# YoungSeng/DiffuseStyleGesture

Hardware: AMD Instinct MI355X
Metric: gesture frames/sec, 1000-step DDPM, 320-frame ZEGGS clip, 1/2/4/8 MI355X (higher is better)
Workload: dtype bf16

## Files before the change

diffusestylegesture_amd/csrc/dsg_fused.h:

```cpp
#pragma once
#include "dsg_kernels.h"

namespace dsg {

struct InLocArgs {
    const void* xs;
    int Jp;
    const void* Wp;
    int KBtot;
    LocArgs loc;
    StepCtl* ctl_upd;
    StepTables st; int n_tab;
};

template <class P, int HD, int W>
__device__ __forceinline__ void inloc_body(const InLocArgs& g) {
    typedef typename P::elem elem;
    constexpr int ES = (int)sizeof(elem);
    preload_kernargs(g);
    const LocArgs& a = g.loc;
    if (blockIdx.z == gridDim.z - 1) {
        if (g.ctl_upd && blockIdx.x == 0 && blockIdx.y == 0 && threadIdx.x == 0) step_advance_B<P>(g.ctl_upd, g.st, g.n_tab);
        return;
    }
// ... 994 lines not shown
#pragma unroll
            for (int e = 0; e < 4; ++e) { pp[e] = f2bf(s[2 * kb][e]); pp[4 + e] = f2bf(s[2 * kb + 1][e]); }
            pfr[kb] = __builtin_bit_cast(f32x4, pp);
        }
    }
    const int q = qt * 16 + lr;
#pragma unroll
    for (int dt = 0; dt < ND; ++dt) {
        f32x4 o = (f32x4){0.f, 0.f, 0.f, 0.f};
#pragma unroll
        for (int kb = 0; kb < NVF; ++kb) o = P::mma(vs[dt * NVF + kb][lane], pfr[kb], o);
        if (q < g.ntok) {
            f32x4 y;
#pragma unroll
            for (int e = 0; e < 4; ++e) y[e] = o[e] * inv;
            P::store4_afrag((elem*)g.out, (size_t)qk_off<P>(b * g.ntok + q, h * HD + dt * 16 + 4 * lg, KD), y);
        }
    }
    DSG_TL_MARK(7);
}

struct FfnArgs {
    const void* A;
    const float* R;
    const void* W1; const float* b1;
    const void* W2; const float* b2;
    const float* ln_g; const float* ln_b;
    float* Xn;
    void* Xa;
    int M, MT;
    const void* Wo; const float* bo;
    const float* ln1_g; const float* ln1_b;
    float* X1;
};

template <class P, int DT, int FT, int RT, int NW, int LA = 2, bool LATE_R = false, bool OP = false, int RING = 0, bool WO_RING = false>
__global__ __launch_bounds__(64 * NW) void k_ffn(const FfnArgs g) {
    DSG_TL_SCOPE();
    typedef typename P::elem elem;
    constexpr int ES = (int)sizeof(elem);
    constexpr int D = 64 * DT, FF = 64 * FT, KD = D / P::KB, KF = FF / P::KB;
    constexpr int FW = FF / 16 / NW, DW = D / 16 / NW;
    constexpr int HP = FF * ES + 16;
    constexpr int KC0 = (DW >= 4 ? 2 : 4) * LA, KC = KC0 < KF ? KC0 : KF, NC = KF / KC;
    constexpr int NT = 64 * NW;
    static_assert(FW >= LA && FW % LA == 0 && DW >= 1 && KF % KC == 0 && (FF / 16) % NW == 0 && (D / 16) % NW == 0, "shape");
    static_assert(!P::W2 || (OP && RING > 0 && RT < 4), "bf16w2: the ring forms with the prologue");
    constexpr int HID_LO = RT * 16 * HP;
    __shared__ __attribute__((aligned(16))) char hid[P::AF * RT * 16 * HP];
    __shared__ float red[RT][2][NW][16];
    __shared__ __attribute__((aligned(16))) float vecs[3][D];
    constexpr int XP = D * ES + 16;
    constexpr bool BIG = OP && RT >= 4;
    constexpr bool X1MEM = BIG || (OP && RT == 2 && D >= 512);
    static_assert(!BIG || RT * 16 * XP <= RT * 16 * HP, "alias");
    constexpr int XA_LO = RT * 16 * XP;
    __shared__ __attribute__((aligned(16))) char xa_own[(OP && !BIG) ? P::AF * RT * 16 * XP : 16];
    char* const xa = BIG ? hid : xa_own;
    __shared__ __attribute__((aligned(16))) float vecs1[OP ? 3 : 1][OP ? D : 4];
    constexpr int X1P = D + 4;
    __shared__ __attribute__((aligned(16))) float x1f[(OP && !X1MEM) ? RT * 16 * X1P : 4];
    preload_kernargs(g);
    const int mb = blockIdx.x;
    const int tid = threadIdx.x, lane = tid & 63, wave = wave_id(), lr = lane & 15, lg = lane >> 4;
    const int m0 = mb * 16 * RT, mt_last = g.MT - 1;
    constexpr int RH = (OP && RT >= 4) ? 2 : RT;
    typename P::afrag af[RT][KD];
    constexpr int NFH = RH * KD, NFW = (NFH + NW - 1) / NW;
    f32x4* const stg = (f32x4*)(hid + P::AF * (RT * 16 * HP - NFH * 1024));
    static_assert(!OP || NFH * 1024 + (RT >= 4 ? RT * 16 * (D * ES + 16) : 0) <= RT * 16 * HP, "the staged fragments sit behind the (aliased) LayerNorm1 rows");
    typename P::afrag afw[OP ? NFW : 1];
    auto load_a = [&](int rt0) {
        if constexpr (OP) {
#pragma unroll
            for (int i = 0; i < NFW; ++i) {
                const int f = min(wave * NFW + i, NFH - 1), rt = rt0 + f / KD, kb = f % KD;
                const int mt = min(mb * RT + rt, mt_last);
                afw[i] = P::aload_frag(g.A, (size_t)(mt * KD + kb), lane);
            }
        } else {
#pragma unroll
            for (int rt = rt0; rt < rt0 + RH; ++rt) {
                const int mt = min(mb * RT + rt, mt_last);
#pragma unroll
                for (int kb = 0; kb < KD; ++kb) af[rt][kb] = P::aload_frag(g.A, (size_t)(mt * KD + kb), lane);
            }
        }
    };
    auto share_a = [&](int rt0) {
#pragma unroll
        for (int i = 0; i < NFW; ++i) if (wave * NFW + i < NFH) {
            if constexpr (P::W2) { stg[((wave * NFW + i) * 2) * 64 + lane] = afw[i].h; stg[((wave * NFW + i) * 2 + 1) * 64 + lane] = afw[i].l; }
            else stg[(wave * NFW + i) * 64 + lane] = afw[i];
        }
        DSG_LDS_BARRIER();
#pragma unroll
        for (int rt = rt0; rt < rt0 + RH; ++rt)
#pragma unroll
            for (int kb = 0; kb < KD; ++kb) af[rt][kb] = P::aload((const char*)&stg[((rt - rt0) * KD + kb) * P::AF * 64 + lane], 1024);
    };
    load_a(0);
    const f32x4* w1 = (const f32x4*)g.W1 + lane;
    const f32x4* w2 = (const f32x4*)g.W2 + lane;
    f32x4 wb1[2][LA][KD], pb1[2][LA];
    auto load1 = [&](int buf, int tp) {
#pragma unroll
        for (int j = 0; j < LA; ++j) {
            const int nt = wave * FW + LA * tp + j;
#pragma unroll
            for (int kb = 0; kb < KD; ++kb) wb1[buf][j][kb] = w1[((size_t)nt * KD + kb) * 64];
            pb1[buf][j] = *(const f32x4*)(g.b1 + nt * 16 + 4 * lg);
        }
    };
    constexpr int N0 = WO_RING ? DW * KD : 0;
    constexpr int N1 = FW * KD, N2 = KF * DW, NRING = RING > 0 ? RING : 1;
    static_assert(RING == 0 || (OP && RING <= N1), "ring");
    static_assert(!WO_RING || (RING > 0 && RING <= N0 && RT <= 2), "W_o in the ring: the 16- and 32-row forms");
    typename P::wfrag ring[NRING];
    const f32x4* wo_ring = (const f32x4*)g.Wo + lane;
    auto ring_load = [&](int ig) -> typename P::wfrag {
        if (ig < N0) return P::wload(wo_ring, (size_t)(wave * DW + ig % DW) * KD + ig / DW);
        const int i = ig - N0;
        if (i < N1) return P::wload(w1, (size_t)(wave * FW + i / KD) * KD + i % KD);
        const int k = (i - N1) / DW, t = (i - N1) % DW;
        return P::wload(w2, (size_t)(wave * DW + t) * KF + k);
    };
    if constexpr (!OP) load1(0, 0);
    f32x4 pr[RT][DW];
    auto rowok_of = [&](int rt) { return m0 + rt * 16 + lr < g.M; };
    auto mrow_of = [&](int rt) { return (unsigned)min(m0 + rt * 16 + lr, g.M - 1); };
#pragma unroll
    for (int rt = 0; rt < RT; ++rt) {
        if ((!LATE_R || OP) && rt < RH) {
#pragma unroll
            for (int t = 0; t < DW; ++t) pr[rt][t] = lda16<P>(g.R, (size_t)((mrow_of(rt) * D + (wave * DW + t) * 16 + 4 * lg) * 4u));
        }
    }
    constexpr int NV = (3 * D / 4 + NT - 1) / NT;
    f32x4 vload[NV], vload1[OP ? NV : 1];
#pragma unroll
    for (int i = 0; i < NV; ++i) {
        const int e = min(tid + NT * i, 3 * D / 4 - 1), vsel = e / (D / 4), vidx = e % (D / 4);
        vload[i] = ((const f32x4*)(vsel == 0 ? g.b2 : (vsel == 1 ? g.ln_g : g.ln_b)))[vidx];
        if constexpr (OP) vload1[i] = ((const f32x4*)(vsel == 0 ? g.bo : (vsel == 1 ? g.ln1_g : g.ln1_b)))[vidx];
    }
    if constexpr (OP) {
        const f32x4* wo = (const f32x4*)g.Wo + lane;
        typename P::wfrag wof[WO_RING ? 1 : DW][WO_RING ? 1 : KD];
        if constexpr (WO_RING) {
#pragma unroll
            for (int i = 0; i < RING; ++i) ring[i] = ring_load(i);
        } else {
#pragma unroll
            for (int t = 0; t < DW; ++t)
#pragma unroll
                for (int kb = 0; kb < KD; ++kb) wof[t][kb] = P::wload(wo, (size_t)(wave * DW + t) * KD + kb);
        }
        DSG_LOADS_ISSUED();
// ... 81 lines not shown
                const int n = (wave * DW + t) * 16 + 4 * lg;
                const f32x4 pg = *(const f32x4*)(&vecs1[1][n]), pbt = *(const f32x4*)(&vecs1[2][n]);
                f32x4 y;
#pragma unroll
                for (int e = 0; e < 4; ++e) y[e] = __builtin_fmaf((acc1[rt][t][e] - mean1[rt]) * rstd, pg[e], pbt[e]);
                P::store4_a((elem*)(xa + (rt * 16 + lr) * XP) + n, XA_LO, y);
                if constexpr (X1MEM) *(f32x4*)((char*)g.X1 + (size_t)(((unsigned)(m0 + rt * 16 + lr) * D + n) * 4u)) = y;
                else *(f32x4*)(x1f + (rt * 16 + lr) * X1P + n) = y;
            }
        }
        if constexpr (RING > 0 && !WO_RING) {
#pragma unroll
            for (int i = 3 * (RING / 4); i < RING; ++i) ring[i] = ring_load(i);
            DSG_LOADS_ISSUED();
        }
        DSG_LDS_BARRIER();
#pragma unroll
        for (int rt = 0; rt < RT; ++rt)
#pragma unroll
            for (int kb = 0; kb < KD; ++kb) af[rt][kb] = P::aload(xa + (rt * 16 + lr) * XP + (kb * P::KB + P::E * lg) * ES, XA_LO);
        if constexpr (BIG) DSG_LDS_BARRIER();
        DSG_TL_MARK(2);
    } else {
        DSG_LOADS_ISSUED();
    }
    f32x4 acc[RT][DW];
#pragma unroll
    for (int rt = 0; rt < RT; ++rt)
#pragma unroll
        for (int t = 0; t < DW; ++t) acc[rt][t] = (f32x4){0.f, 0.f, 0.f, 0.f};
    if constexpr (RING > 0) {
        static_assert(OP, "ring: the forms with the prologue");
        f32x4 pbr[2];
        pbr[0] = *(const f32x4*)(g.b1 + (wave * FW) * 16 + 4 * lg);
#pragma unroll
        for (int j = 0; j < FW; ++j) {
            const int nt = wave * FW + j;
            if (j + 1 < FW) pbr[(j + 1) & 1] = *(const f32x4*)(g.b1 + (nt + 1) * 16 + 4 * lg);
            f32x4 c[RT];
#pragma unroll
            for (int rt = 0; rt < RT; ++rt) c[rt] = (f32x4){0.f, 0.f, 0.f, 0.f};
#pragma unroll
            for (int kb = 0; kb < KD; ++kb) {
                const int i = N0 + j * KD + kb;
#pragma unroll
                for (int rt = 0; rt < RT; ++rt) c[rt] = P::mma_w(ring[i % NRING], af[rt][kb], c[rt]);
                if (i + RING < N0 + N1 + N2) ring[i % NRING] = ring_load(i + RING);
                DSG_LOADS_ISSUED();
            }
#pragma unroll
            for (int rt = 0; rt < RT; ++rt) {
                f32x4 y;
#pragma unroll
                for (int e = 0; e < 4; ++e) y[e] = gelu_erf<P>(c[rt][e] + pbr[j & 1][e]);
                P::store4_a((elem*)(hid + (rt * 16 + lr) * HP) + nt * 16 + 4 * lg, HID_LO, y);
            }
        }
        if constexpr (X1MEM) {
            int lr_late = lr;
#ifndef DSG_EMU
            asm volatile("" : "+v"(lr_late));
#endif
#pragma unroll
            for (int rt = 0; rt < RT; ++rt)
#pragma unroll
                for (int t = 0; t < DW; ++t) pr[rt][t] = lda16<P>((const float*)g.X1, (size_t)(((unsigned)(m0 + rt * 16 + lr_late) * D + (wave * DW + t) * 16 + 4 * lg) * 4u));
        }
        DSG_TL_MARK(3);
        DSG_LDS_BARRIER();
        DSG_TL_MARK(4);
        constexpr int AB = RT <= 2 ? 2 : 1;
        typename P::afrag a[AB][RT];
        if constexpr (AB == 2) {
#pragma unroll
            for (int rt = 0; rt < RT; ++rt) a[0][rt] = P::aload(hid + (rt * 16 + lr) * HP + (P::E * lg) * ES, HID_LO);
        }
#pragma unroll
        for (int k = 0; k < KF; ++k) {
            if (AB == 1 || k + 1 < KF) {
                const int kn = AB == 2 ? k + 1 : k;
#pragma unroll
                for (int rt = 0; rt < RT; ++rt) a[kn % AB][rt] = P::aload(hid + (rt * 16 + lr) * HP + (kn * P::KB + P::E * lg) * ES, HID_LO);
            }
#pragma unroll
            for (int t = 0; t < DW; ++t) {
                const int i = N0 + N1 + k * DW + t;
#pragma unroll
                for (int rt = 0; rt < RT; ++rt) acc[rt][t] = P::mma_w(ring[i % NRING], a[k % AB][rt], acc[rt][t]);
                if (i + RING < N0 + N1 + N2) ring[i % NRING] = ring_load(i + RING);
            }
            DSG_LOADS_ISSUED();
        }
    } else {
    #pragma unroll
        for (int tp = 0; tp < FW / LA; ++tp) {
            if (tp + 1 < FW / LA) { load1((tp + 1) & 1, tp + 1); DSG_LOADS_ISSUED(); }
    #pragma unroll
            for (int j = 0; j < LA; ++j) {
                const int nt = wave * FW + LA * tp + j;
    #pragma unroll
                for (int rt = 0; rt < RT; ++rt) {
                    f32x4 c = (f32x4){0.f, 0.f, 0.f, 0.f};
    #pragma unroll
                    for (int kb = 0; kb < KD; ++kb) c = P::mma(wb1[tp & 1][j][kb], af[rt][kb], c);
                    f32x4 y;
    #pragma unroll
                    for (int e = 0; e < 4; ++e) y[e] = gelu_erf<P>(c[e] + pb1[tp & 1][j][e]);
                    P::store4((elem*)(hid + (rt * 16 + lr) * HP) + nt * 16 + 4 * lg, y);
                }
            }
        }
// ... 13 lines not shown
    #endif
            }
    #pragma unroll
            for (int rt = 0; rt < RT; ++rt) {
                const unsigned mr = X1MEM ? (unsigned)(m0 + rt * 16 + lr_late) : (unsigned)min(m0 + rt * 16 + lr_late, g.M - 1);
    #pragma unroll
                for (int t = 0; t < DW; ++t) pr[rt][t] = lda16<P>(X1MEM ? (const float*)g.X1 : g.R, (size_t)((mr * D + (wave * DW + t) * 16 + 4 * lg) * 4u));
            }
        }
        DSG_LOADS_ISSUED();
        if constexpr (!OP) {
    #pragma unroll
            for (int i = 0; i < NV; ++i) {
                const int e = tid + NT * i;
                if (e < 3 * D / 4) *(f32x4*)(&vecs[0][0] + e * 4) = vload[i];
            }
        }
        DSG_LDS_BARRIER();
    #pragma unroll
        for (int c = 0; c < NC; ++c) {
            if (c + 1 < NC) { load2((c + 1) & 1, c + 1); DSG_LOADS_ISSUED(); }
    #pragma unroll
            for (int k = 0; k < KC; ++k) {
    #pragma unroll
                for (int rt = 0; rt < RT; ++rt) {
                    const f32x4 a = *(const f32x4*)(hid + (rt * 16 + lr) * HP + ((c * KC + k) * P::KB + P::E * lg) * ES);
    #pragma unroll
                    for (int t = 0; t < DW; ++t) acc[rt][t] = P::mma(wb2[c & 1][k][t], a, acc[rt][t]);
                }
            }
        }
    }
    DSG_TL_MARK(5);
#pragma unroll
    for (int rt = 0; rt < RT; ++rt) {
        float sm = 0.f;
#pragma unroll
        for (int t = 0; t < DW; ++t) {
            const f32x4 pb = *(const f32x4*)(&vecs[0][(wave * DW + t) * 16 + 4 * lg]);
            if constexpr (OP && !X1MEM) pr[rt][t] = *(const f32x4*)(x1f + (rt * 16 + lr) * X1P + (wave * DW + t) * 16 + 4 * lg);
            acc[rt][t] = acc[rt][t] + pb + pr[rt][t];
            sm += (acc[rt][t][0] + acc[rt][t][1]) + (acc[rt][t][2] + acc[rt][t][3]);
        }
        ln_wave_moments<DW>(acc[rt], sm, red[rt][0][wave], red[rt][1][wave], lr, lg);
    }
    DSG_LDS_BARRIER();
    float mean[RT];
    float var2[RT];
#pragma unroll
    for (int rt = 0; rt < RT; ++rt) ln_combine_moments<NW, D>(red[rt][0], red[rt][1], lr, mean[rt], var2[rt]);
#pragma unroll
    for (int rt = 0; rt < RT; ++rt) {
        const float rstd = 1.0f / sqrtf(var2[rt] + 1e-5f);
        if (rowok_of(rt)) {
#pragma unroll
            for (int t = 0; t < DW; ++t) {
                const int n = (wave * DW + t) * 16 + 4 * lg;
                const f32x4 pg = *(const f32x4*)(&vecs[1][n]), pbt = *(const f32x4*)(&vecs[2][n]);
                f32x4 y;
#pragma unroll
                for (int e = 0; e < 4; ++e) y[e] = __builtin_fmaf((acc[rt][t][e] - mean[rt]) * rstd, pg[e], pbt[e]);
                *(f32x4*)((char*)g.Xn + (size_t)((mrow_of(rt) * D + n) * 4u)) = y;
                P::store4_afrag((elem*)g.Xa, (size_t)qk_off<P>((int)mrow_of(rt), n, KD), y);
            }
        }
    }
    DSG_TL_MARK(6);
}

struct FfnPartArgs {
    const void* A;
    const void* W1; const float* b1;
    const void* W2;
    float* part;
// ... 259 lines not shown
```

diffusestylegesture_amd/csrc/dsg_hip.cpp:

```cpp
#include "dsg_fused.h"
#include "dsg_batched.h"
#include "dsg_stream.h"
#include "../../include/dsg.h"
#include "dsg_aql.h"

#include <algorithm>
#include <atomic>
#include <cmath>
#include <cstdio>
#include <cstdlib>
#include <cstring>
#include <map>
#include <memory>
#include <mutex>
#include <string>
#include <tuple>
#include <vector>

using namespace dsg;

static thread_local std::string g_err;
static int fail(int code, const std::string& msg) { g_err = msg; return code; }
#define HIPCHK(expr)                                                                                     \
    do {                                                                                                 \
// ... 76 lines not shown
struct dsg_handle {
    dsg_config cfg;
    int prec = 0, es = 4, kbk = 16;
    int J, T, S, D, As, A, W, L, H, hd, ff, Hl, hdl, ntok, Tp, Jp, Jq, Bmax, Ta, n_te;
    int KSin = 4;
    hipStream_t stream = nullptr;
    hipEvent_t ev_in = nullptr, ev_out = nullptr, ev_t0 = nullptr, ev_t1 = nullptr;
    std::vector<void*> allocs;
    std::vector<void*> allocs_uc;
    std::shared_ptr<SharedWeights> shared;
    bool alloc_shared = false;
    bool is_clone = false;
    std::map<std::string, RawT> raw;
    bool finalized = false, cond_set = false;
    int condB = 0;
    void* Wp_in = nullptr; void* Wp_out = nullptr; float* b_out = nullptr;
    std::vector<Layer> layers;
    float *TE = nullptr, *TE2 = nullptr, *rcos = nullptr, *rsin = nullptr, *cbase = nullptr, *zero_bias = nullptr;
    float *emb1 = nullptr, *Cf = nullptr, *enc = nullptr, *cvec = nullptr;
    float *c_style = nullptr, *c_seed = nullptr, *c_audio = nullptr, *c_seed_last = nullptr;
    int seed_last_B = 0;
    unsigned char* mask = nullptr; int mb = 1; int nomask = 0;
    int cfgB = 0; float* cfg_scale = nullptr;
    int last_path = -1;
    bool last_nofence = false;
    int kset_req = DSG_KSET_AUTO;
    int last_kset = -1;
    float *xs32 = nullptr, *partial = nullptr, *X0 = nullptr, *pre1 = nullptr, *pre2 = nullptr, *Xn = nullptr,
          *X1 = nullptr, *fwd_out = nullptr, *io_tmp = nullptr, *io_tmp2 = nullptr, *ext_noise = nullptr;
    size_t ext_noise_cap = 0;
    void *xsA = nullptr, *X0a = nullptr, *q = nullptr, *k = nullptr, *vt = nullptr, *attn = nullptr, *hidden = nullptr;
    int lanes_now = 1;
    float* ffn_part = nullptr; size_t ffn_slab = 0;
    void* X1a = nullptr;
    int* ctr = nullptr;
    StepCtl* ctl = nullptr;
    int* t_arr = nullptr; unsigned* dyn = nullptr;
    int latency_mode = -1;
#ifndef DSG_EMU
    dsg_aql::Ctx aql;
#endif
    int uc_mode = 1;
    bool alloc_uc = false;
    bool state_fences = false;
    int fence_next = 0;
    int aql_mode = 1;
    bool aql_warned = false;
    bool aql_timing = false;
    double aql_ms = 0.0;
    int env_loc64_from = 2048;
    int env_ffn_rt4 = -1;
    int env_ffn_split = -1;
    int env_clip_attn = -1;
    int* st_tmodel = nullptr; float* st_c[5] = {nullptr, nullptr, nullptr, nullptr, nullptr};
    int st_cap = 0, n_run = 1;
    bool st_valid = false; int st_mode = -1, st_skip = -1; float st_eta = 0.f;
    Sched sched;
    struct GKey { int B, mode, mb, cn, n_run, n_tab, flags, kset; bool operator<(const GKey& o) const {
        return std::tie(B, mode, mb, cn, n_run, n_tab, flags, kset) < std::tie(o.B, o.mode, o.mb, o.cn, o.n_run, o.n_tab, o.flags, o.kset); } };
    struct GVal { hipGraphExec_t exec; hipGraph_t graph; int steps; };
    std::map<GKey, GVal> graphs;
    float last_ms = -1.f; int last_steps = 0; bool timing_valid = false;
};

static inline bool is_bf16(const dsg_handle* h) { return h->prec != DSG_PREC_FP32; }

struct UcArena {
    char* base = nullptr; size_t size = 0, used = 0;
    std::map<size_t, size_t> free;
    bool quarantined = false;
};
struct UcPool {
    std::mutex mu;
    std::vector<UcArena> arenas[64];
    std::map<void*, std::pair<char*, size_t>> live;
    size_t trimmed = 0;
    static size_t cap_bytes() { const char* e = getenv("DSG_UC_POOL_CAP_MB"); return (size_t)(e ? std::max(atoll(e), 0ll) : 16384ll) << 20; }
};
static UcPool& uc_pool() { static UcPool* p = new UcPool(); return *p; }
constexpr size_t UC_ALIGN = 4096, UC_ARENA_MIN = (size_t)32 << 20, UC_ARENA_GRAN = (size_t)2 << 20;
#ifndef DSG_EMU
__global__ void k_uc_fill(unsigned* p, size_t n, unsigned salt) {
    for (size_t i = (size_t)blockIdx.x * blockDim.x + threadIdx.x; i < n; i += (size_t)gridDim.x * blockDim.x) p[i] = (unsigned)i * 2654435761u + salt;
}
__global__ void k_uc_verify(const unsigned* p, size_t n, unsigned salt, unsigned* bad) {
    unsigned b = 0;
// ... 225 lines not shown
    h->cfg = *c;
    h->prec = c->precision;
    h->es = is_bf16(h) ? 2 : 4;
    h->kbk = is_bf16(h) ? 32 : 16;
    h->J = c->njoints; h->T = c->n_poses; h->S = c->n_seed; h->D = c->latent_dim; h->As = c->audio_src_dim;
    h->A = c->audio_dim; h->W = c->window; h->L = c->num_layers; h->H = c->num_heads; h->hd = hd; h->ff = c->ff_size;
    h->Hl = c->local_heads; h->hdl = hdl; h->ntok = ntok; h->Tp = Tp;
    h->Jp = rup(h->J, 128); h->Jq = rup(h->J, 4); h->Bmax = c->max_batch;
    h->KSin = cdiv(h->Jp, 256);
    h->Ta = c->variant == 3 ? h->T : h->T - h->S * (c->variant == 5 ? 2 : 1);
    h->n_te = c->train_steps > 0 ? c->train_steps : 1000;
    if (h->n_te > c->pe_max_len) { delete h; return fail(DSG_E_INVALID, "train_steps > pe_max_len"); }
    h->layers.resize(h->L);
    h->latency_mode = c->latency_mode == 1 ? 0 : (c->latency_mode == 2 ? 1 : -1);
    if (const char* e = getenv("DSG_KSET")) {
        char* end = nullptr;
        const long v = strtol(e, &end, 10);
        if (end == e || *end != 0 || v < DSG_KSET_AUTO || v > DSG_KSET_ROWS) {
            delete h;
            return fail(DSG_E_INVALID, std::string("DSG_KSET must be 0 (auto) .. 5 (rows), got '") + e + "'");
        }
        h->kset_req = (int)v;
    }
    if (c->max_batch > 16 && !stream_set_ok(h) && !rows_w2_ok(h)) h->uc_mode = 0;
    if (const char* e = getenv("DSG_UC")) h->uc_mode = atoi(e);
    if (const char* e = getenv("DSG_AQL")) h->aql_mode = atoi(e);
    else {
        for (const char* v : {"ROCP_TOOL_LIBRARIES", "HSA_TOOLS_LIB", "ROCPROFILER_REGISTER_FORCE_LOAD", "ROCPROF_COUNTER_COLLECTION", "ROCPROF_KERNEL_TRACE", "LD_PRELOAD"}) {
            const char* val = getenv(v);
            if (val && (strstr(val, "rocprof") || strstr(v, "ROCPROF"))) h->aql_mode = 0;
        }
    }
    if (const char* e = getenv("DSG_FFN_RT4")) h->env_ffn_rt4 = std::max(atoi(e), 0);
    if (const char* e = getenv("DSG_LOC64_FROM")) h->env_loc64_from = std::max(atoi(e), 1);
    if (const char* e = getenv("DSG_FFN_SPLIT")) h->env_ffn_split = atoi(e) != 0 ? 1 : 0;
    if (const char* e = getenv("DSG_CLIP_ATTN")) h->env_clip_attn = atoi(e) != 0 ? 1 : 0;
    *out = h;

    HIPCHK(hipStreamCreateWithFlags(&h->stream, hipStreamNonBlocking));
    HIPCHK(hipEventCreateWithFlags(&h->ev_in, hipEventDisableTiming));
    HIPCHK(hipEventCreateWithFlags(&h->ev_out, hipEventDisableTiming));
    HIPCHK(hipEventCreate(&h->ev_t0));
    HIPCHK(hipEventCreate(&h->ev_t1));

    const int B = h->Bmax, D = h->D;
    const size_t Min_pad = rup(B * h->T, 16) + 16 + 128, M_pad = rup(B * ntok, 16) + Tp + 128;
    h->state_fences = h->uc_mode == 1 && !(getenv("DSG_STATE_UC") && atoi(getenv("DSG_STATE_UC")));
    h->alloc_uc = !h->state_fences;
    CHK(dalloc(h, &h->xs32, (size_t)B * h->T * h->Jp + 16 * h->Jp));
    if (is_bf16(h)) CHK(dalloc_bytes(h, &h->xsA, ((size_t)Min_pad * h->Jp) * h->es));
    h->alloc_uc = true;
    CHK(dalloc(h, &h->partial, (size_t)h->KSin * Min_pad * D));
    CHK(dalloc(h, &h->X0, M_pad * D));
    CHK(dalloc_bytes(h, &h->X0a, M_pad * D * h->es * (h->prec == DSG_PREC_BF16W2 ? 2 : 1)));
    CHK(dalloc(h, &h->pre1, M_pad * D));
    CHK(dalloc(h, &h->pre2, M_pad * D));
    CHK(dalloc(h, &h->Xn, M_pad * D));
    CHK(dalloc(h, &h->X1, M_pad * D));
    CHK(dalloc_bytes(h, &h->attn, M_pad * D * h->es * (h->prec == DSG_PREC_BF16W2 ? 2 : 1)));
    CHK(dalloc_bytes(h, &h->X1a, M_pad * D * h->es));
    CHK(dalloc_bytes(h, &h->hidden, M_pad * (size_t)h->ff * h->es * (h->prec == DSG_PREC_BF16W2 ? 2 : 1)));
    h->ffn_slab = M_pad * D;
    const size_t qkv_elems = (size_t)B * h->H * Tp * hd;
    CHK(dalloc_bytes(h, &h->q, qkv_elems * h->es));
    CHK(dalloc_bytes(h, &h->k, qkv_elems * h->es));
    CHK(dalloc_bytes(h, &h->vt, qkv_elems * h->es));
// ... 322 lines not shown
            HIPCHK(hipMemcpyAsync(h->c_seed_last + (size_t)B * h->J * h->S, h->c_seed_last, (size_t)B * h->J * h->S * sizeof(float),
                                  hipMemcpyDeviceToDevice, h->stream));
        CHK(cond_rows(h, style, seed, audio, B, B, 1));
        CHK(upload(h, h->cfg_scale, cfg_scale, (size_t)B * sizeof(float)));
    }
    h->cfgB = cfg_scale ? B : 0;
    h->cond_set = true;
    h->condB = rows;
    CHK(order_before(h, stream));
    return 0;
}
extern "C" int dsg_set_window_cond(dsg_handle* h, const float* style, const float* seed, const float* audio,
                                   const uint8_t* mask_local, int mask_batch, int B, int uncond, void* stream) {
    return set_window_cond(h, style, seed, audio, mask_local, mask_batch, B, uncond, nullptr, stream);
}
extern "C" int dsg_set_window_cond_cfg(dsg_handle* h, const float* style, const float* seed, const float* audio,
                                       const uint8_t* mask_local, int mask_batch, int B, const float* scale, void* stream) {
    if (!scale) return fail(DSG_E_INVALID, "dsg_set_window_cond_cfg: scale required (y['scale'])");
    return set_window_cond(h, style, seed, audio, mask_local, mask_batch, B, 0, scale, stream);
}

struct KernelSel {
    int set = DSG_KSET_TILE;
    bool lat = false;
    bool attn_in_mid = false;
    bool blk = false;
    bool attn_op = false;
    bool stream = false;
    bool ffn = false;
    bool ffn16_wide = false;
    bool clip_w = false;
    bool ffn_rt2w = false;
    bool ffn16 = false;
    bool ffn_rt4 = false;
    bool ffn_split = false;
    bool clip_attn = false;
    bool xs_frag = false;
};
static bool have_attn_mid(const dsg_handle* h, int B) {
    return B == 1 && h->H == 4 && ((h->D == 256 && h->Tp == 96) || (h->D == 128 && h->Tp == 32));
}
static bool have_attn_op_narrow(const dsg_handle* h) {
    return h->prec == DSG_PREC_BF16 && h->H == 4 && ((h->D == 256 && h->Tp == 96) || (h->D == 128 && h->Tp == 32));
}
static bool have_attn_op_wide(const dsg_handle* h) {
    if (h->H != 4 || h->prec == DSG_PREC_BF16W2) return false;
    if (h->prec == DSG_PREC_BF16) return (h->D == 384 || h->D == 512) && h->Tp == 160;
    return (h->D == 256 && h->Tp == 96) || (h->D == 128 && h->Tp == 32);
}
static bool have_attn_op(const dsg_handle* h) { return have_attn_op_narrow(h) || have_attn_op_wide(h); }
static bool latency_set_ok(const dsg_handle* h) {
    const int dt = h->D / 64;
    return h->D <= 256 && (dt == 1 || dt == 2 || dt == 4);
}
static bool stream_set_ok(const dsg_handle* h) {
    return have_attn_op_narrow(h) && (h->D == 256 || h->D == 128) && (h->ff == 1024 || h->ff == 128) && (h->Jp == 1152 || h->Jp == 128);
}
static bool ffn_split_wide(const dsg_handle* h) {
    if (h->prec == DSG_PREC_FP32) return have_attn_op_wide(h) && h->ff == 1024 && h->D == 256;
    return h->prec == DSG_PREC_BF16 && have_attn_op_wide(h) && h->ff == 1024 && (h->D == 384 || h->D == 512);
}
static bool ffn_split_ok(const dsg_handle* h) { return stream_set_ok(h) || ffn_split_wide(h); }
static bool rows_wide_ok(const dsg_handle* h) {
    return h->prec == DSG_PREC_BF16 && h->H == 4 && h->Tp == 160 && h->ff == 1024 && (h->D == 384 || h->D == 512);
}
static bool rows_w2_ok(const dsg_handle* h) {
// ... 43 lines not shown
        return fail(DSG_E_NOT_IMPLEMENTED, "precision bf16w2: kernel sets LATENCY (latent_dim <= 256), TILE and ROWS (latent_dim 128 / 256) only");
    k = KernelSel();
    k.set = set;
    k.lat = set == DSG_KSET_LATENCY;
    k.attn_in_mid = k.lat && have_attn_mid(h, B);
    k.stream = set == DSG_KSET_STREAM;
    k.ffn = k.stream;
    k.ffn16 = set == DSG_KSET_ROWS;
    if (k.ffn16) k.ffn = true;
    {
        const int rows = B * h->ntok, e = h->env_ffn_rt4;
        k.ffn_rt4 = k.ffn && (e >= 0 ? (e > 0 && rows >= e) : (h->lanes_now >= 4 && rows >= 4000));
    }
    k.blk = set == DSG_KSET_BLOCK || set == DSG_KSET_ROWS || k.stream;
    if (k.ffn16 && h->prec == DSG_PREC_BF16W2 && h->cfgB > 0) return fail(DSG_E_NOT_IMPLEMENTED, "precision bf16w2, kernel set ROWS: no fused guidance (TILE has it)");
    k.attn_op = !k.lat && (have_attn_op_narrow(h) || (k.blk && have_attn_op_wide(h)) || (k.ffn16 && rows_w2_ok(h)));
    k.ffn16_wide = k.ffn16 && rows_wide_ok(h);
    if (k.ffn16_wide) {
#if !defined(DSG_X_NO_CLIP_W)
        k.clip_w = h->H == 4 && h->Tp == 160;
#endif
#if defined(DSG_X_FFN_RT2W)
        k.ffn_rt2w = DSG_X_FFN_RT2W != 0;
#else
        k.ffn_rt2w = h->lanes_now >= 3 && h->lanes_now * cdiv(B * h->ntok, 16) > 256;
#endif
        if (h->cfgB > 0) return fail(DSG_E_NOT_IMPLEMENTED, "kernel set ROWS at the DSG+ widths: no fused guidance (BLOCK has it)");
        k.attn_op = false;
    }
    k.xs_frag = k.blk && h->prec == DSG_PREC_BF16 && (h->Jp == 1152 || h->Jp == 128 || xs_frag_wide(h, set));
    if (set == DSG_KSET_BLOCK && ffn_split_ok(h)) k.ffn_split = h->env_ffn_split != 0;
    k.clip_attn = (k.ffn_split || k.ffn) && have_attn_op_narrow(h) && h->env_clip_attn != 0;
    if (k.ffn16 && h->prec == DSG_PREC_BF16W2) k.clip_attn = true;

    return 0;
}

static int ensure_set_buffers(dsg_handle* h, const KernelSel& k) {
    if (k.ffn_split && !h->ffn_part) {
        const bool was = h->alloc_uc;
        h->alloc_uc = true;
        const int rc = dalloc(h, &h->ffn_part, (size_t)(ffn_split_wide(h) ? 8 : 4) * h->ffn_slab);
        h->alloc_uc = was;
        if (rc) return rc;
    }
    return 0;
}

extern "C" int dsg_set_kernel_set(dsg_handle* h, int set) {
    if (!h) return fail(DSG_E_INVALID, "null handle");
    if (set < DSG_KSET_AUTO || set > DSG_KSET_ROWS) return fail(DSG_E_INVALID, "dsg_set_kernel_set: unknown kernel set");
    if (set == DSG_KSET_LATENCY && h->D > 512) return fail(DSG_E_NOT_IMPLEMENTED, "kernel set LATENCY: latent_dim > 512");
    if ((set == DSG_KSET_STREAM || set == DSG_KSET_ROWS) && !stream_set_ok(h) && !(set == DSG_KSET_ROWS && (rows_w2_ok(h) || rows_wide_ok(h))))
        return fail(DSG_E_NOT_IMPLEMENTED, "kernel sets STREAM / ROWS: bf16 (ROWS: bf16w2 as well), latent_dim 128 / 256, 4 heads, ff 128 / 1024 only");
    if (h->prec == DSG_PREC_BF16W2 && ((set > DSG_KSET_TILE && !(set == DSG_KSET_ROWS && rows_w2_ok(h))) || (set == DSG_KSET_LATENCY && h->D > 256)))
        return fail(DSG_E_NOT_IMPLEMENTED, "precision bf16w2: kernel sets LATENCY (latent_dim <= 256), TILE and ROWS (latent_dim 128 / 256) only");
    if (getenv("DSG_KSET")) {
        static std::atomic<bool> said{false};
        if (set != h->kset_req && !said.exchange(true))
            fprintf(stderr, "libdsg_hip: WARNING: DSG_KSET=%s pins the kernel set of every handle; dsg_set_kernel_set(%d) ignored "
                            "(dsg_get_kernel_set reports the set in force)\n", getenv("DSG_KSET"), set);
        return 0;
    }
    h->kset_req = set;
    return 0;
}
extern "C" int dsg_get_kernel_set(dsg_handle* h, int* set) {
    if (!h || !set) return fail(DSG_E_INVALID, "null argument");
    *set = h->kset_req;
    return 0;
}
extern "C" int dsg_recommend_kernel_set(dsg_handle* h, int B, int lanes, int* set) {
    if (!h || !set || B <= 0 || lanes <= 0) return fail(DSG_E_INVALID, "dsg_recommend_kernel_set: bad argument");
    *set = resolve_auto_set(h, B, lanes);
    return 0;
}
extern "C" int dsg_last_kernel_set(dsg_handle* h, int* set) {
// ... 345 lines not shown
                CHK((launch_gemm_w<P, PRO_LN, EPI_QKV>(h, g, ks)));
            }
        }
        if (!ks.attn_in_mid && !ks.attn_op && !clip_w_done) {
            AttnArgs a;
            memset(&a, 0, sizeof(a));
            a.q = h->q; a.k = h->k; a.vt = h->vt; a.out = h->attn; a.B = B; a.H = h->H; a.ntok = ntok; a.Tp = h->Tp;
            a.D = D;
            CHK(launch_attn<P>(h, a));
        }
        if (ks.lat) {
            MidArgs a;
            memset(&a, 0, sizeof(a));
            a.A = h->attn; a.R = l == 0 ? h->X0 : h->Xn; a.Wo = ly.Wo; a.bo = ly.bo; a.ln_g = ly.g1; a.ln_b = ly.be1;
            a.W1 = ly.W1; a.b1 = ly.b1; a.X1 = h->X1; a.hidden = h->hidden; a.M = M; a.MT = MT; a.ff = h->ff;
            if (ks.attn_in_mid) {
                AttnMidArgs am;
                am.mid = a; am.q = h->q; am.k = h->k; am.vt = h->vt; am.ntok = ntok; am.Tp = h->Tp;
                CHK(launch_attn_mid<P>(h, am));
            } else {
                CHK(launch_mid<P>(h, a));
            }
        } else if (ks.attn_op) {
          if constexpr (P::W2) {
            if (!clip_l || !ks.ffn16) return fail(DSG_E_NOT_IMPLEMENTED, "precision bf16w2: k_clip_attn + k_ffn in the ROWS set only");
            ClipAttnArgs a;
            a.X = h->X0a; a.Wqkv = ly.Wqkv; a.bqkv = ly.bqkv; a.out = h->attn; a.B = B; a.ntok = ntok;
            if (D == 256) CHK((step_launch<&k_clip_attn<P, 4, 6>>(h, dim3(4, B), dim3(384), a)));
            else CHK((step_launch<&k_clip_attn<P, 2, 2>>(h, dim3(4, B), dim3(128), a)));
            FfnArgs f;
            memset(&f, 0, sizeof(f));
            f.W1 = ly.W1; f.b1 = ly.b1; f.W2 = ly.W2; f.b2 = ly.b2; f.ln_g = ly.g2; f.ln_b = ly.be2; f.Xn = h->Xn; f.Xa = h->X0a; f.M = M; f.MT = MT;
            f.A = h->attn; f.R = l == 0 ? h->X0 : h->Xn; f.Wo = ly.Wo; f.bo = ly.bo; f.ln1_g = ly.g1; f.ln1_b = ly.be1; f.X1 = h->X1;
            if (D == 256) CHK((step_launch<&k_ffn<P, 4, 16, 1, 8, 2, true, true, 12>>(h, dim3(MT), dim3(512), f)));
            else CHK((step_launch<&k_ffn<P, 2, 2, 1, 4, 2, false, true, 8>>(h, dim3(MT), dim3(256), f)));
            continue;
          } else {
            if (clip_l) {
                if constexpr (sizeof(typename P::elem) == 2) {
                    ClipAttnArgs a;
                    a.X = h->X0a; a.Wqkv = ly.Wqkv; a.bqkv = ly.bqkv; a.out = h->attn; a.B = B; a.ntok = ntok;
                    if (D == 256) CHK((step_launch<&k_clip_attn<P, 4, 6>>(h, dim3(4, B), dim3(384), a)));
                    else CHK((step_launch<&k_clip_attn<P, 2, 2>>(h, dim3(4, B), dim3(128), a)));
                }
            } else {
                AttnOpArgs a;
                a.q = h->q; a.k = h->k; a.vt = h->vt; a.R = l == 0 ? h->X0 : h->Xn; a.Wo = ly.Wo; a.bo = ly.bo; a.ln_g = ly.g1; a.ln_b = ly.be1;
                a.X1 = h->X1; a.X1a = h->X1a; a.B = B; a.ntok = ntok; a.Tp = h->Tp;
                const dim3 grid(cdiv(ntok, 16), B);
                if constexpr (sizeof(typename P::elem) == 2) {
                    if (D == 256 && h->Tp == 96) CHK((step_launch<&k_attn_op<P, 4, 6>>(h, grid, dim3(256), a)));
                    else if (D == 128 && h->Tp == 32) CHK((step_launch<&k_attn_op<P, 2, 2>>(h, grid, dim3(256), a)));
                    else if (D == 384) CHK((step_launch<&k_attn_op_w<P, 6, 10>>(h, grid, dim3(256), a)));
                    else CHK((step_launch<&k_attn_op_w<P, 8, 10>>(h, grid, dim3(256), a)));
                } else {
                    if (D == 256) CHK((step_launch<&k_attn_op_w<P, 4, 6>>(h, grid, dim3(256), a)));
                    else CHK((step_launch<&k_attn_op_w<P, 2, 2>>(h, grid, dim3(256), a)));
                }
            }
            if (ks.ffn && !(h->cfgB > 0 && l == h->L - 1)) {
                FfnArgs a;
                memset(&a, 0, sizeof(a));
                a.A = h->X1a; a.R = h->X1; a.W1 = ly.W1; a.b1 = ly.b1; a.W2 = ly.W2; a.b2 = ly.b2; a.ln_g = ly.g2; a.ln_b = ly.be2;
                a.Xn = h->Xn; a.Xa = h->X0a; a.M = M; a.MT = MT;
                if (clip_l) {
                    a.A = h->attn; a.R = l == 0 ? h->X0 : h->Xn; a.Wo = ly.Wo; a.bo = ly.bo; a.ln1_g = ly.g1; a.ln1_b = ly.be1; a.X1 = h->X1;
                }
// ... 345 lines not shown
    return 0;
}

extern "C" int dsg_forward(dsg_handle* h, const float* x, const int64_t* t, float* out, int B, void* stream) {
    if (!h || !x || !t || !out) return fail(DSG_E_INVALID, "dsg_forward: null argument");
    if (!h->finalized || !h->cond_set) return fail(DSG_E_STATE, "dsg_forward before finalize / set_window_cond");
    int rows = 0;
    CHK(rows_for(h, B, &rows));
    HIPCHK(hipSetDevice(h->cfg.device));
    CHK(order_after(h, stream));
    std::vector<int> tt(rows);
    if (is_device_ptr(t)) {
        std::vector<int64_t> th(B);
        HIPCHK(hipMemcpy(th.data(), t, B * sizeof(int64_t), hipMemcpyDeviceToHost));
        for (int i = 0; i < B; ++i) tt[i] = (int)th[i];
    } else {
        for (int i = 0; i < B; ++i) tt[i] = (int)t[i];
    }
    for (int i = B; i < rows; ++i) tt[i] = tt[i - B];
    for (int i = 0; i < B; ++i)
        if (tt[i] < 0 || tt[i] >= h->n_te) return fail(DSG_E_INVALID, "timestep out of range");
    HIPCHK(hipMemcpyAsync(h->t_arr, tt.data(), rows * sizeof(int), hipMemcpyHostToDevice, h->stream));
    HIPCHK(hipStreamSynchronize(h->stream));
    const size_t n = (size_t)B * h->J * h->T;
    const float* xd = nullptr;
    CHK(to_dev(h, x, h->io_tmp, n, &xd));
    NoiseKey nk = {0, 0, 0, 0};
    StepCtx c; c.B = rows; c.out_mode = OUT_FORWARD; c.use_ctr = false; c.ext_noise = nullptr; c.const_noise = 0;
    CHK(select_kernels(h, rows, c.ks));
    CHK(ensure_set_buffers(h, c.ks));
    CHK(launch_x_in(h, xd, nullptr, 0, 0.f, 0.f, 0, nk, 0, B, c.ks));
    CHK(run_step_p(h, c));
    CHK(from_dev(h, out, h->fwd_out, n));
    CHK(order_before(h, stream));
    return 0;
}

static int build_step_tables(dsg_handle* h, int mode, int skip, float eta, int* n_run_out) {
    const Sched& s = h->sched;
    if (s.n == 0) return fail(DSG_E_STATE, "dsg_sample before dsg_set_schedule");
    if (skip < 0 || skip >= s.n) return fail(DSG_E_INVALID, "skip_timesteps out of range");
    const int n_run = s.n - skip;
    if (h->st_valid && h->st_mode == mode && h->st_skip == skip && h->st_eta == eta) {
        *n_run_out = n_run; h->n_run = n_run;
        return 0;
    }
    std::vector<int> tm(n_run);
    std::vector<float> c[5];
    for (auto& v : c) v.assign(n_run, 0.f);
    for (int i = 0; i < n_run; ++i) {
        const int idx = n_run - 1 - i;
        tm[i] = s.tmap[idx];
        const float nz = idx == 0 ? 0.f : 1.f;
        if (mode == DSG_MODE_DDPM) {
            c[0][i] = (float)s.coef1[idx];
            c[1][i] = (float)s.coef2[idx];
            c[2][i] = nz * expf(0.5f * (float)s.plogvar[idx]);
        } else {
            const float ab = (float)s.ac[idx], abp = (float)s.acp[idx];
            const float sigma = eta * sqrtf((1.f - abp) / (1.f - ab)) * sqrtf(1.f - ab / abp);
            c[0][i] = (float)s.sqrt_recip[idx];
            c[1][i] = (float)s.sqrt_recipm1[idx];
            c[2][i] = sqrtf(abp);
            c[3][i] = sqrtf(1.f - abp - sigma * sigma);
            c[4][i] = nz * sigma;
        }
// ... 142 lines not shown
    if (h->aql_mode == 1 && !job.dumping && !graph_wanted && n_run > 0) {
        bool planned = dsg_aql::init(h->aql, h->cfg.device, (const void*)&dsg_version);
        bool nofence = false;
        if (planned && h->uc_mode == 1) nofence = uc_selfcheck(h);
        HP_LAP(3);
        if (planned) {
            dsg_aql::begin(h->aql);
            const int rc = run_step_p(h, c);
            HP_LAP(4);
            planned = dsg_aql::finish(h->aql) && rc == 0;
            HP_LAP(5);
            h->aql.recording = false;
            h->aql.nofence = nofence;
        }
        if (!planned) {
            if (!h->aql_warned) { fprintf(stderr, "libdsg_hip: AQL path unavailable (%s); using HIP launches\n", h->aql.err.c_str()); h->aql_warned = true; }
            h->aql_mode = 0;
        } else {
            HIPCHK(hipStreamSynchronize(h->stream));
            job.aql = true;
        }
    }
#endif
    HIPCHK(hipEventRecord(h->ev_t0, h->stream));
    HP_LAP(6);
    return 0;
}

static int sample_run_hip(dsg_handle* h, const dsg_sample_args* a, SampleJob& job) {
    const int n_run = job.n_run, B = job.B, spg = job.spg;
    const StepCtx& c = job.c;
    const size_t n = (size_t)B * h->J * h->T;
    if (spg > 0 && n_run >= spg && job.done == 0) {
        dsg_handle::GKey key = {c.B, c.out_mode, h->mb, c.const_noise, n_run, h->n_run, (c.clip_x0 ? 1 : 0) | (h->cfgB ? 2 : 0) | (h->nomask ? 4 : 0) | (c.ks.attn_in_mid ? 8 : 0) | (c.no_noise ? 16 : 0),
                                c.ks.set};
        auto it = h->graphs.find(key);
        bool ok = true;
        if (it == h->graphs.end()) {
            hipGraph_t graph = nullptr;
            hipGraphExec_t exec = nullptr;
            hipError_t e = hipStreamBeginCapture(h->stream, hipStreamCaptureModeThreadLocal);
            if (e == hipSuccess) {
                int rc = 0;
                for (int s = 0; s < spg && rc == 0; ++s) rc = run_step_p(h, c);
                e = hipStreamEndCapture(h->stream, &graph);
                if (rc != 0 || e != hipSuccess || !graph) ok = false;
                if (ok && hipGraphInstantiate(&exec, graph, nullptr, nullptr, 0) != hipSuccess) ok = false;
            } else ok = false;
            if (!ok) { (void)hipGetLastError(); if (graph) (void)hipGraphDestroy(graph); }
            else {
                dsg_handle::GVal v = {exec, graph, spg};
                it = h->graphs.emplace(key, v).first;
            }
        }
        if (ok) {
            while (n_run - job.done >= spg) { HIPCHK(hipGraphLaunch(it->second.exec, h->stream)); job.done += spg; }
            h->last_path = 2;
            h->last_kset = c.ks.set;
        }
    }
    int di = 0;
    for (; job.done < n_run; ++job.done) {
        CHK(run_step_p(h, c));
        if (job.dumping) {
            while (di < a->n_dump && a->dump_steps[di] < job.first + job.done) ++di;
            if (di < a->n_dump && a->dump_steps[di] == job.first + job.done) {
                CHK(launch_x_out(h, h->fwd_out, B));
// ... 187 lines not shown
```

Measured before the change: 734.4.

## Split D=256 fused FFN hidden dimension across two blocks with atomic-counter reduction

Adds a HALF=2 variant of the fused FFN kernel where each 16-row tile is processed by two blocks, each covering half of the hidden (FF) dimension. The two partial W2 results are exchanged through an uncached global slab, and a per-tile atomic counter picks the second-arriving block to finish the residual add and LayerNorm. It is enabled when the doubled grid fits in 256 blocks, so small-batch cases can fill more CUs at the cost of a global-memory handoff and fences. A HALF=1 variant folds the bias and residual into the accumulator midway through the loop, and the graph cache key gains the new kernel-set flags.

```diff
diff --git a/diffusestylegesture_amd/csrc/dsg_fused.h b/diffusestylegesture_amd/csrc/dsg_fused.h
--- a/diffusestylegesture_amd/csrc/dsg_fused.h
+++ b/diffusestylegesture_amd/csrc/dsg_fused.h
@@ -1050,16 +1050,20 @@
     const void* Wo; const float* bo;
     const float* ln1_g; const float* ln1_b;
     float* X1;
+    float* slab;
+    int* cnt;
 };
 
-template <class P, int DT, int FT, int RT, int NW, int LA = 2, bool LATE_R = false, bool OP = false, int RING = 0, bool WO_RING = false>
+template <class P, int DT, int FT, int RT, int NW, int LA = 2, bool LATE_R = false, bool OP = false, int RING = 0, bool WO_RING = false, int HALF = 0>
 __global__ __launch_bounds__(64 * NW) void k_ffn(const FfnArgs g) {
     DSG_TL_SCOPE();
     typedef typename P::elem elem;
     constexpr int ES = (int)sizeof(elem);
-    constexpr int D = 64 * DT, FF = 64 * FT, KD = D / P::KB, KF = FF / P::KB;
+    constexpr int D = 64 * DT, FFW = 64 * FT, KD = D / P::KB, KFW = FFW / P::KB;
+    constexpr int FF = HALF == 2 ? FFW / 2 : FFW, KF = FF / P::KB;
     constexpr int FW = FF / 16 / NW, DW = D / 16 / NW;
     constexpr int HP = FF * ES + 16;
+    static_assert(HALF == 0 || (OP && RT == 1 && RING > 0 && !WO_RING && KFW % 2 == 0), "HALF: the 16-row ring form with the prologue");
     constexpr int KC0 = (DW >= 4 ? 2 : 4) * LA, KC = KC0 < KF ? KC0 : KF, NC = KF / KC;
     constexpr int NT = 64 * NW;
     static_assert(FW >= LA && FW % LA == 0 && DW >= 1 && KF % KC == 0 && (FF / 16) % NW == 0 && (D / 16) % NW == 0, "shape");
@@ -1079,7 +1083,12 @@
     constexpr int X1P = D + 4;
     __shared__ __attribute__((aligned(16))) float x1f[(OP && !X1MEM) ? RT * 16 * X1P : 4];
     preload_kernargs(g);
-    const int mb = blockIdx.x;
+    int mb = blockIdx.x, hh = 0;
+    if constexpr (HALF == 2) {
+        const int q = (int)blockIdx.x / 16, r = (int)blockIdx.x % 16, G = min(8, g.MT - 8 * q);
+        mb = 8 * q + r % G;
+        hh = r / G;
+    }
     const int tid = threadIdx.x, lane = tid & 63, wave = wave_id(), lr = lane & 15, lg = lane >> 4;
     const int m0 = mb * 16 * RT, mt_last = g.MT - 1;
     constexpr int RH = (OP && RT >= 4) ? 2 : RT;
@@ -1120,6 +1129,7 @@
     load_a(0);
     const f32x4* w1 = (const f32x4*)g.W1 + lane;
     const f32x4* w2 = (const f32x4*)g.W2 + lane;
+    const int nt1 = hh * (FF / 16), k2 = hh * KF;
     f32x4 wb1[2][LA][KD], pb1[2][LA];
     auto load1 = [&](int buf, int tp) {
 #pragma unroll
@@ -1139,9 +1149,9 @@
     auto ring_load = [&](int ig) -> typename P::wfrag {
         if (ig < N0) return P::wload(wo_ring, (size_t)(wave * DW + ig % DW) * KD + ig / DW);
         const int i = ig - N0;
-        if (i < N1) return P::wload(w1, (size_t)(wave * FW + i / KD) * KD + i % KD);
+        if (i < N1) return P::wload(w1, (size_t)(nt1 + wave * FW + i / KD) * KD + i % KD);
         const int k = (i - N1) / DW, t = (i - N1) % DW;
-        return P::wload(w2, (size_t)(wave * DW + t) * KF + k);
+        return P::wload(w2, (size_t)(wave * DW + t) * KFW + k2 + k);
     };
     if constexpr (!OP) load1(0, 0);
     f32x4 pr[RT][DW];
@@ -1289,11 +1299,11 @@
     if constexpr (RING > 0) {
         static_assert(OP, "ring: the forms with the prologue");
         f32x4 pbr[2];
-        pbr[0] = *(const f32x4*)(g.b1 + (wave * FW) * 16 + 4 * lg);
+        pbr[0] = *(const f32x4*)(g.b1 + (nt1 + wave * FW) * 16 + 4 * lg);
 #pragma unroll
         for (int j = 0; j < FW; ++j) {
             const int nt = wave * FW + j;
-            if (j + 1 < FW) pbr[(j + 1) & 1] = *(const f32x4*)(g.b1 + (nt + 1) * 16 + 4 * lg);
+            if (j + 1 < FW) pbr[(j + 1) & 1] = *(const f32x4*)(g.b1 + (nt1 + nt + 1) * 16 + 4 * lg);
             f32x4 c[RT];
 #pragma unroll
             for (int rt = 0; rt < RT; ++rt) c[rt] = (f32x4){0.f, 0.f, 0.f, 0.f};
@@ -1334,6 +1344,16 @@
         }
 #pragma unroll
         for (int k = 0; k < KF; ++k) {
+            if constexpr (HALF == 1) {
+                if (k == KF / 2) {
+#pragma unroll
+                    for (int t = 0; t < DW; ++t) {
+                        const int n = (wave * DW + t) * 16 + 4 * lg;
+                        pr[0][t] = acc[0][t] + *(const f32x4*)(&vecs[0][n]) + *(const f32x4*)(x1f + lr * X1P + n);
+                        acc[0][t] = (f32x4){0.f, 0.f, 0.f, 0.f};
+                    }
+                }
+            }
             if (AB == 1 || k + 1 < KF) {
                 const int kn = AB == 2 ? k + 1 : k;
 #pragma unroll
@@ -1413,14 +1433,52 @@
         }
     }
     DSG_TL_MARK(5);
+    if constexpr (HALF == 2) {
+        f32x4* const slab = (f32x4*)g.slab + (size_t)mb * (2 * NW * DW * 64) + lane;
+#pragma unroll
+        for (int t = 0; t < DW; ++t) {
+            if (hh == 0) {
+                const int n = (wave * DW + t) * 16 + 4 * lg;
+                acc[0][t] = acc[0][t] + *(const f32x4*)(&vecs[0][n]) + *(const f32x4*)(x1f + lr * X1P + n);
+            }
+            slab[(hh * NW * DW + wave * DW + t) * 64] = acc[0][t];
+        }
+#ifndef DSG_EMU
+        asm volatile("s_waitcnt vmcnt(0)" ::: "memory");
+#endif
+        __syncthreads();
+        if (tid == 0) {
+            __builtin_amdgcn_fence(__ATOMIC_RELEASE, "agent");
+#ifndef DSG_EMU
+            asm volatile("s_waitcnt vmcnt(0)" ::: "memory");
+#endif
+            const int prev = __hip_atomic_fetch_add(&g.cnt[mb], 1, __ATOMIC_RELAXED, __HIP_MEMORY_SCOPE_AGENT);
+            if (prev == 1) {
+                __builtin_amdgcn_fence(__ATOMIC_ACQUIRE, "agent");
+#ifndef DSG_EMU
+                asm volatile("s_waitcnt vmcnt(0)" ::: "memory");
+#endif
+                __hip_atomic_store(&g.cnt[mb], 0, __ATOMIC_RELAXED, __HIP_MEMORY_SCOPE_AGENT);
+            }
+            vecs1[0][0] = prev == 1 ? 1.f : 0.f;
+        }
+        __syncthreads();
+        if (vecs1[0][0] == 0.f) return;
+#pragma unroll
+        for (int t = 0; t < DW; ++t) acc[0][t] = acc[0][t] + slab[((1 - hh) * NW * DW + wave * DW + t) * 64];
+    }
 #pragma unroll
     for (int rt = 0; rt < RT; ++rt) {
         float sm = 0.f;
 #pragma unroll
         for (int t = 0; t < DW; ++t) {
-            const f32x4 pb = *(const f32x4*)(&vecs[0][(wave * DW + t) * 16 + 4 * lg]);
-            if constexpr (OP && !X1MEM) pr[rt][t] = *(const f32x4*)(x1f + (rt * 16 + lr) * X1P + (wave * DW + t) * 16 + 4 * lg);
-            acc[rt][t] = acc[rt][t] + pb + pr[rt][t];
+            if constexpr (HALF == 1) {
+                acc[rt][t] = pr[rt][t] + acc[rt][t];
+            } else if constexpr (HALF == 0) {
+                const f32x4 pb = *(const f32x4*)(&vecs[0][(wave * DW + t) * 16 + 4 * lg]);
+                if constexpr (OP && !X1MEM) pr[rt][t] = *(const f32x4*)(x1f + (rt * 16 + lr) * X1P + (wave * DW + t) * 16 + 4 * lg);
+                acc[rt][t] = acc[rt][t] + pb + pr[rt][t];
+            }
             sm += (acc[rt][t][0] + acc[rt][t][1]) + (acc[rt][t][2] + acc[rt][t][3]);
         }
         ln_wave_moments<DW>(acc[rt], sm, red[rt][0][wave], red[rt][1][wave], lr, lg);
diff --git a/diffusestylegesture_amd/csrc/dsg_hip.cpp b/diffusestylegesture_amd/csrc/dsg_hip.cpp
--- a/diffusestylegesture_amd/csrc/dsg_hip.cpp
+++ b/diffusestylegesture_amd/csrc/dsg_hip.cpp
@@ -132,6 +132,7 @@
     void *xsA = nullptr, *X0a = nullptr, *q = nullptr, *k = nullptr, *vt = nullptr, *attn = nullptr, *hidden = nullptr;
     int lanes_now = 1;
     float* ffn_part = nullptr; size_t ffn_slab = 0;
+    float* ffn_half = nullptr; int* ffn_cnt = nullptr;
     void* X1a = nullptr;
     int* ctr = nullptr;
     StepCtl* ctl = nullptr;
@@ -152,6 +153,9 @@
     int env_ffn_rt4 = -1;
     int env_ffn_split = -1;
     int env_clip_attn = -1;
+#ifdef DSG_EMU
+    int emu_ffn_half2 = -1;
+#endif
     int* st_tmodel = nullptr; float* st_c[5] = {nullptr, nullptr, nullptr, nullptr, nullptr};
     int st_cap = 0, n_run = 1;
     bool st_valid = false; int st_mode = -1, st_skip = -1; float st_eta = 0.f;
@@ -443,6 +447,9 @@
         }
     }
     if (const char* e = getenv("DSG_FFN_RT4")) h->env_ffn_rt4 = std::max(atoi(e), 0);
+#ifdef DSG_EMU
+    if (const char* e = getenv("DSG_EMU_FFN_HALF2")) h->emu_ffn_half2 = atoi(e) != 0;
+#endif
     if (const char* e = getenv("DSG_LOC64_FROM")) h->env_loc64_from = std::max(atoi(e), 1);
     if (const char* e = getenv("DSG_FFN_SPLIT")) h->env_ffn_split = atoi(e) != 0 ? 1 : 0;
     if (const char* e = getenv("DSG_CLIP_ATTN")) h->env_clip_attn = atoi(e) != 0 ? 1 : 0;
@@ -831,6 +838,7 @@
     bool clip_w = false;
     bool ffn_rt2w = false;
     bool ffn16 = false;
+    bool ffn_half2 = false;
     bool ffn_rt4 = false;
     bool ffn_split = false;
     bool clip_attn = false;
@@ -940,6 +948,16 @@
     if (set == DSG_KSET_BLOCK && ffn_split_ok(h)) k.ffn_split = h->env_ffn_split != 0;
     k.clip_attn = (k.ffn_split || k.ffn) && have_attn_op_narrow(h) && h->env_clip_attn != 0;
     if (k.ffn16 && h->prec == DSG_PREC_BF16W2) k.clip_attn = true;
+    if (k.ffn16 && h->D == 256 && h->prec == DSG_PREC_BF16W2) {
+#if defined(DSG_X_FFN_HALF2)
+        k.ffn_half2 = DSG_X_FFN_HALF2 != 0;
+#else
+        k.ffn_half2 = h->lanes_now * 2 * cdiv(B * h->ntok, 16) <= 256;
+#endif
+#ifdef DSG_EMU
+        if (h->emu_ffn_half2 >= 0) k.ffn_half2 = h->emu_ffn_half2 != 0;
+#endif
+    }
 
     return 0;
 }
@@ -951,6 +969,17 @@
         const int rc = dalloc(h, &h->ffn_part, (size_t)(ffn_split_wide(h) ? 8 : 4) * h->ffn_slab);
         h->alloc_uc = was;
         if (rc) return rc;
+    }
+    if (k.ffn_half2) {
+        if (!h->ffn_half) {
+            const bool was = h->alloc_uc;
+            h->alloc_uc = true;
+            int rc = dalloc(h, &h->ffn_half, 2 * h->ffn_slab);
+            h->alloc_uc = was;
+            if (!rc) rc = dalloc(h, &h->ffn_cnt, h->ffn_slab / ((size_t)16 * h->D));
+            if (rc) return rc;
+        }
+        HIPCHK(hipMemsetAsync(h->ffn_cnt, 0, h->ffn_slab / ((size_t)16 * h->D) * sizeof(int), h->stream));
     }
     return 0;
 }
@@ -1362,7 +1391,9 @@
             memset(&f, 0, sizeof(f));
             f.W1 = ly.W1; f.b1 = ly.b1; f.W2 = ly.W2; f.b2 = ly.b2; f.ln_g = ly.g2; f.ln_b = ly.be2; f.Xn = h->Xn; f.Xa = h->X0a; f.M = M; f.MT = MT;
             f.A = h->attn; f.R = l == 0 ? h->X0 : h->Xn; f.Wo = ly.Wo; f.bo = ly.bo; f.ln1_g = ly.g1; f.ln1_b = ly.be1; f.X1 = h->X1;
-            if (D == 256) CHK((step_launch<&k_ffn<P, 4, 16, 1, 8, 2, true, true, 12>>(h, dim3(MT), dim3(512), f)));
+            f.slab = h->ffn_half; f.cnt = h->ffn_cnt;
+            if (D == 256 && ks.ffn_half2) CHK((step_launch<&k_ffn<P, 4, 16, 1, 8, 2, true, true, 12, false, 2>>(h, dim3(2 * MT), dim3(512), f)));
+            else if (D == 256) CHK((step_launch<&k_ffn<P, 4, 16, 1, 8, 2, true, true, 12, false, 1>>(h, dim3(MT), dim3(512), f)));
             else CHK((step_launch<&k_ffn<P, 2, 2, 1, 4, 2, false, true, 8>>(h, dim3(MT), dim3(256), f)));
             continue;
           } else {
@@ -1774,6 +1805,13 @@
     CHK(launch_x_in(h, xd, nullptr, 0, 0.f, 0.f, 0, nk, 0, B, c.ks));
     CHK(run_step_p(h, c));
     CHK(from_dev(h, out, h->fwd_out, n));
+#ifdef DSG_EMU
+    if (c.ks.ffn_half2) {
+        std::vector<int> cnt(h->ffn_slab / ((size_t)16 * h->D));
+        HIPCHK(hipMemcpy(cnt.data(), h->ffn_cnt, cnt.size() * sizeof(int), hipMemcpyDeviceToHost));
+        for (int v : cnt) if (v != 0) return fail(DSG_E_STATE, "k_ffn<HALF = 2>: a row tile's counter was left non-zero");
+    }
+#endif
     CHK(order_before(h, stream));
     return 0;
 }
@@ -1982,7 +2020,8 @@
     const StepCtx& c = job.c;
     const size_t n = (size_t)B * h->J * h->T;
     if (spg > 0 && n_run >= spg && job.done == 0) {
-        dsg_handle::GKey key = {c.B, c.out_mode, h->mb, c.const_noise, n_run, h->n_run, (c.clip_x0 ? 1 : 0) | (h->cfgB ? 2 : 0) | (h->nomask ? 4 : 0) | (c.ks.attn_in_mid ? 8 : 0) | (c.no_noise ? 16 : 0),
+        dsg_handle::GKey key = {c.B, c.out_mode, h->mb, c.const_noise, n_run, h->n_run, (c.clip_x0 ? 1 : 0) | (h->cfgB ? 2 : 0) | (h->nomask ? 4 : 0) | (c.ks.attn_in_mid ? 8 : 0) | (c.no_noise ? 16 : 0)
+                                | (c.ks.ffn_half2 ? 32 : 0) | (c.ks.ffn_rt2w ? 64 : 0) | (c.ks.ffn_rt4 ? 128 : 0),
                                 c.ks.set};
         auto it = h->graphs.find(key);
         bool ok = true;
```

Result: no change. 744.9 (median of 6 runs) (+1.4%).
